# mratsim/constantine

Hardware: NVIDIA H100
Metric: bls12_381_g1_msm_throughput (higher is better)
Workload: dtype u32

## Files before the change

constantine_b200/csrc/msm_affine.cuh:

```cuda
#pragma once
#include "ec.cuh"
#include "field_inv.cuh"

namespace b200 {

constexpr int AFF_MAX_LEVELS = 8;
constexpr uint32_t AFF_NONE = 0xFFFFFFFFu;

static __global__ void k_bucket_bounds(const uint32_t* __restrict__ keys, size_t n, uint32_t no_key, uint32_t* head, uint32_t* tail) {
  size_t q = (size_t)blockIdx.x * blockDim.x + threadIdx.x;
  if (q >= n) return;
  const uint32_t key = keys[q];
  if (key >= no_key) return;
  if (q == 0 || keys[q - 1] != key) head[key] = (uint32_t)q;
  if (q + 1 == n || keys[q + 1] != key) tail[key] = (uint32_t)(q + 1);
}

constexpr int SCAN_THREADS = 256, SCAN_PER_THREAD = 4, SCAN_ITEMS = SCAN_THREADS * SCAN_PER_THREAD;

B200_DEV uint32_t block_exclusive_scan(uint32_t v, uint32_t& total, uint32_t* smem ) {
  const unsigned lane = threadIdx.x & 31u, warp = threadIdx.x >> 5;
  uint32_t inc = v;
#pragma unroll
  for (int d = 1; d < 32; d <<= 1) {
// ... 254 lines not shown
  else load_words_rw(x, src + (size_t)ref * (2 * T::WORDS));
  return x;
}
template <class T, bool FIRST>
B200_DEV T load_y(const uint32_t* src, uint32_t ref, bool& is_inf_if_x_zero) {
  T y;
  if constexpr (FIRST) {
    load_words(y, src + (size_t)(ref & 0x7FFFFFFFu) * (2 * T::WORDS) + T::WORDS);
    is_inf_if_x_zero = y.is_zero();
    y.cneg((ref >> 31) != 0);
  } else {
    load_words_rw(y, src + (size_t)ref * (2 * T::WORDS) + T::WORDS);
    is_inf_if_x_zero = y.is_zero();
  }
  return y;
}

template <class T>
B200_DEV int classify_pair(bool single, const T& x1, const T& y1, bool inf1, const T& x2, const T& y2, bool inf2, T& den) {
  if (single) return PAIR_COPY1;
  if (inf1) return PAIR_COPY2;
  if (inf2) return PAIR_COPY1;
  den = x2 - x1;
  if (!den.is_zero()) return PAIR_ADD;
  if (!(y1 == y2) || y1.is_zero()) return PAIR_INF;
  den = y1.dbl();
  return PAIR_DBL;
}

#ifndef B200_AFF_THREADS
#define B200_AFF_THREADS 128
#endif
#ifndef B200_AFF_MIN_BLOCKS
#define B200_AFF_MIN_BLOCKS 4
#endif

B200_DEV void prefetch_l2(const void* p) { asm volatile("prefetch.global.L2 [%0];" ::"l"(p)); }
B200_DEV void prefetch_span(const void* p, int bytes) {
  prefetch_l2(p);
  prefetch_l2((const char*)p + bytes - 1);
}
template <class T, bool FIRST>
B200_DEV void prefetch_point(const uint32_t* src, uint32_t ref) {
  const uint32_t idx = FIRST ? (ref & 0x7FFFFFFFu) : ref;
  prefetch_span(src + (size_t)idx * (2 * T::WORDS), 2 * T::WORDS * 4);
}

template <class T, bool FIRST>
__global__ void __launch_bounds__(B200_AFF_THREADS, (T::WORDS <= 12) ? B200_AFF_MIN_BLOCKS : 1)
k_affine_pairs(const void* __restrict__ plan, const uint32_t* __restrict__ total_ptr, const uint32_t* src, uint32_t* dst, uint4* scratch,
               const uint32_t* __restrict__ perm = nullptr, const uint32_t* __restrict__ range = nullptr) {
  const size_t threads = (size_t)gridDim.x * blockDim.x;
  const size_t tid = (size_t)blockIdx.x * blockDim.x + threadIdx.x;
  const uint32_t range_begin = range ? range[0] : 0u;
  const uint32_t total = range ? range[1] - range[0] : *total_ptr;
  if (perm) perm += range_begin;
  const uint32_t M = (uint32_t)(((size_t)total + threads - 1) / threads);
  const unsigned lane = threadIdx.x & 31u;
  const size_t warp_base = (tid - lane) * (size_t)M;
  if (warp_base >= total) return;
  uint32_t cnt = 0;
  {
    const size_t first = warp_base + lane;
    if (first < total) {
      const size_t left = (size_t)total - first;
      cnt = (uint32_t)((left + 31) / 32);
      if (cnt > M) cnt = M;
    }
  }
  T run = T::one();
  {
    auto slot_of = [&](size_t t) -> size_t { return perm ? (size_t)perm[t] : t; };
    PairTask t_next = cnt ? load_task<FIRST>(plan, slot_of(warp_base + lane)) : PairTask{0u, AFF_NONE};
    T x1n = T::zero(), x2n = T::zero();
    if (cnt) {
      x1n = load_x<T, FIRST>(src, t_next.a);
      if (t_next.b != AFF_NONE) x2n = load_x<T, FIRST>(src, t_next.b);
    }
#pragma unroll 1
    for (uint32_t j = 0; j < cnt; j++) {
      const PairTask t = t_next;
      const T x1 = x1n, x2 = x2n;
      if (j + 1 < cnt) {
        t_next = load_task<FIRST>(plan, slot_of(warp_base + lane + 32u * (size_t)(j + 1)));
        x1n = load_x<T, FIRST>(src, t_next.a);
        if (t_next.b != AFF_NONE) x2n = load_x<T, FIRST>(src, t_next.b);
      }
      const bool single = t.b == AFF_NONE;
      T den = x2 - x1;
      bool contributes = !single;
      if (!single && (den.is_zero() || x1.is_zero() || x2.is_zero())) {
        bool z1, z2;
        const T y1 = load_y<T, FIRST>(src, t.a, z1), y2 = load_y<T, FIRST>(src, t.b, z2);
        const int kind = classify_pair(false, x1, y1, z1 && x1.is_zero(), x2, y2, z2 && x2.is_zero(), den);
        contributes = kind >= PAIR_ADD;
      }
      if (contributes) run = run.mul_u(den);
      scratch_store(scratch, threads, tid, j, run);
    }
  }
  T inv = fe_inverse(run);
  auto slot_of2 = [&](size_t t) -> size_t { return perm ? (size_t)perm[t] : t; };
  size_t p_prev = cnt ? slot_of2(warp_base + lane + 32u * (size_t)(cnt - 1)) : 0;
  PairTask t_prev = cnt ? load_task<FIRST>(plan, p_prev) : PairTask{0u, AFF_NONE};
#pragma unroll 1
  for (uint32_t jj = cnt; jj > 0; jj--) {
    const uint32_t j = jj - 1;
    const size_t p = p_prev;
    const PairTask t = t_prev;
    if (j > 0) {
      p_prev = slot_of2(warp_base + lane + 32u * (size_t)(j - 1));
      t_prev = load_task<FIRST>(plan, p_prev);
      prefetch_point<T, FIRST>(src, t_prev.a);
      if (t_prev.b != AFF_NONE) prefetch_point<T, FIRST>(src, t_prev.b);
      if (j > 1) {
        constexpr int V = T::WORDS / 4;
#pragma unroll
        for (int k = 0; k < V; k++) prefetch_l2(scratch + ((size_t)(j - 2) * V + k) * threads + tid);
      }
    }
    const bool single = t.b == AFF_NONE;
    Aff<T> P1, P2;
    bool z1 = false, z2 = false;
    P1.x = load_x<T, FIRST>(src, t.a);
    P1.y = load_y<T, FIRST>(src, t.a, z1);
    if (!single) {
      P2.x = load_x<T, FIRST>(src, t.b);
      P2.y = load_y<T, FIRST>(src, t.b, z2);
    } else {
      P2.x = T::zero(); P2.y = T::zero();
    }
    T den;
    const int kind = classify_pair(single, P1.x, P1.y, z1 && P1.x.is_zero(), P2.x, P2.y, z2 && P2.x.is_zero(), den);
    Aff<T> R;
    if (kind < PAIR_ADD) {
      if (kind == PAIR_COPY1) R = P1;
      else if (kind == PAIR_COPY2) R = P2;
      else { R.x = T::zero(); R.y = T::zero(); }
    } else {
      T inv_den = inv;
      if (j > 0) inv_den = inv.mul_u(scratch_load<T>(scratch, threads, tid, j - 1));
      inv = inv.mul_u(den);
      T num;
      if (kind == PAIR_ADD) num = P2.y - P1.y;
      else { const T xx = P1.x.sqr(); num = xx.dbl() + xx; }
      const T lam = num.mul_u(inv_den);
      R.x = lam.sqr_u() - P1.x - P2.x;
      R.y = lam.mul_u(P1.x - R.x) - P1.y;
    }
    store_affine(dst, p, R);
  }
}

}
```

constantine_b200/csrc/msm_engine.cuh:

```cuda
#pragma once
#include <cstdio>
#include <cstdlib>
#include <cstring>
#include <atomic>
#include <condition_variable>
#include <functional>
#include <memory>
#include <mutex>
#include <thread>
#include <vector>
#include <cuda_runtime.h>
#include <cub/device/device_radix_sort.cuh>
#include <cub/device/device_scan.cuh>
#include "msm_kernels.cuh"
#include "msm_affine.cuh"
#include "host_field.hpp"

namespace b200 {

#define B200_CUDA_CHECK(expr)                                                                              \
  do {                                                                                                     \
    cudaError_t e__ = (expr);                                                                              \
    if (e__ != cudaSuccess) {                                                                              \
      fprintf(stderr, "[ctt_b200_msm] FATAL CUDA error %s (%s) at %s:%d -- no CPU fallback exists\n",      \
// ... 347 lines not shown
                                      const PointChunks* point_chunks = nullptr, bool batch_out_device = false) {
  using T = typename C::T;
  using H = typename C::H;
  using HP = host::HXyzz<H>;
  constexpr int KFIX = 32;
  Stats& st = E.stats;
  int launches = 0;
  if (batch == 0) return HP::inf();
  if (n == 0) {
    if (batch_out) for (size_t m = 0; m < batch; m++) batch_out[m] = HP::inf();
    return HP::inf();
  }
  if (batch * n >= (1ull << 31)) { fprintf(stderr, "[ctt_b200_msm] FATAL: len >= 2^31 unsupported\n"); abort(); }
  if (batch > 1 && (batch_out == nullptr || win_begin != 0 || win_end >= 0 || point_sets < 1 || point_sets > batch)) {
    fprintf(stderr, "[ctt_b200_msm] FATAL: a batch takes all windows and needs an output array\n"); abort();
  }
  const bool table_mode = table_stride > 0;
  if (input_chunks && (batch > 1 || table_mode || input_chunks->empty())) input_chunks = nullptr;

  int c = force_c > 0 ? force_c : (E.tuning.force_c > 0 ? E.tuning.force_c : choose_window(n, C::SCALAR_BITS, T::WORDS));
  if (c < 2) c = 2;
  if (c > 20) c = 20;
  DigitPlan plan = make_plan(C::SCALAR_BITS, c, win_begin, win_end);
  const int nwd = plan.win_end - plan.win_begin;
  if (nwd <= 0) return HP::inf();
  const int nws = table_mode ? 1 : nwd;
  const size_t nw_total = batch * (size_t)nws;
  if (table_mode && (size_t)nwd * table_stride >= (1ull << 31)) { fprintf(stderr, "[ctt_b200_msm] FATAL: table too large\n"); abort(); }
  const uint32_t B = plan.buckets_per_window;
  const size_t nbuckets = nw_total * B;
  if (nbuckets >= 0xFFFFFFF0ull || nw_total >= (1ull << 30) || (size_t)nwd * batch * n >= (1ull << 32)) {
    fprintf(stderr, "[ctt_b200_msm] FATAL: batch too large for 32-bit bucket keys\n"); abort();
  }
  const int nw = (int)nw_total;
  const uint32_t no_key = (uint32_t)nbuckets;
  constexpr size_t XYZZ_BYTES = 4 * T::WORDS * 4;
  constexpr size_t XW = 4 * T::WORDS;
  constexpr size_t AFF_BYTES = 2 * T::WORDS * 4;
  st.c = c; st.num_windows = nwd; st.total_buckets = nbuckets; st.ms_affine = 0; st.entries = 0; st.groups = 1;
#ifndef B200_INLINE_MAX_WORDS
#define B200_INLINE_MAX_WORDS 12
#endif
  constexpr bool INL = (T::WORDS <= B200_INLINE_MAX_WORDS);
  cudaStream_t s = E.compute();
  E.buckets.ensure(nbuckets * XYZZ_BYTES);
  if (E.collect_timing) B200_CUDA_CHECK(cudaEventRecord(E.ev[0], s));
  B200_CUDA_CHECK(cudaMemsetAsync(E.buckets.ptr, 0, nbuckets * XYZZ_BYTES, s));

  const std::vector<InputChunk> whole = {InputChunk{0, n, wait_points}};
  const std::vector<InputChunk>& chunks_in = input_chunks ? *input_chunks : whole;
  for (size_t ck = 0; ck < chunks_in.size(); ck++) {
    const InputChunk& ch = chunks_in[ck];
    if (ch.count == 0) continue;
    const bool into = ck > 0;
    const bool last_chunk = ck + 1 == chunks_in.size();
    const bool timed = E.collect_timing && last_chunk;
    const size_t nper = ch.count;
    const size_t ntot = batch * nper;
    const size_t entries = (size_t)nwd * ntot;
    const void* sc = (const char*)d_scalars + ch.begin * 32;
    const void* pts = table_mode ? d_points : (const void*)((const char*)d_points + ch.begin * AFF_BYTES);
    st.entries += entries;

    int AL = E.tuning.affine_levels;
    if (AL < 0) AL = auto_affine_levels(entries, nbuckets, batch, T::WORDS);
    if (entries >= (1ull << 31) || nbuckets >= (1ull << 30)) AL = 0;
    if (AL > AFF_MAX_LEVELS) AL = AFF_MAX_LEVELS;
    auto level_cap = [&](int r) { return (entries >> r) + nbuckets + 1; };
    const size_t acc_entries = AL ? level_cap(AL) : entries;
    int KACC = 64;
    uint32_t fit_threads;
    {
      static thread_local int acc_bps_cache[MAX_DEVICES] = {};
      int bps = acc_bps_cache[E.device];
      if (bps == 0) {
        B200_CUDA_CHECK(cudaOccupancyMaxActiveBlocksPerMultiprocessor(&bps, k_accumulate<T>, B200_ACC_THREADS, 0));
        if (bps < 1) bps = 1;
        acc_bps_cache[E.device] = bps;
      }
      fit_threads = (uint32_t)(E.sm_count * bps * B200_ACC_THREADS);
      if (E.tuning.slice_len > 0) { KACC = E.tuning.slice_len; fit_threads = 0; }
      else if (E.tuning.slice_len < 0) KACC = -E.tuning.slice_len;
    }
    st.slice_len = fit_threads ? accumulate_slice_len(acc_entries, fit_threads, KACC) : KACC;
    E.keys_a.ensure(entries * 4); E.keys_b.ensure(entries * 4);
    E.vals_a.ensure(entries * 4); E.vals_b.ensure(entries * 4);
    if (timed) B200_CUDA_CHECK(cudaEventRecord(E.ev[10], s));
    if (input_chunks && ch.ready) B200_CUDA_CHECK(cudaStreamWaitEvent(s, ch.ready, 0));
    {
      dim3 grid((unsigned)((ntot + 255) / 256)), block(256);
      const uint32_t msm_key_stride = (uint32_t)nws * B, psets = batch > 1 ? (uint32_t)point_sets : 1u;
      if (fr_mont)
        k_digits<typename C::FrParams, true><<<grid, block, 0, s>>>((const uint32_t*)sc, (uint32_t)ntot, plan, (uint32_t*)E.keys_a.ptr, (uint32_t*)E.vals_a.ptr,
                                                                     table_mode ? 0u : B, no_key, (uint32_t)table_stride, (uint32_t)nper, msm_key_stride, psets);
      else
        k_digits<typename C::FrParams, false><<<grid, block, 0, s>>>((const uint32_t*)sc, (uint32_t)ntot, plan, (uint32_t*)E.keys_a.ptr, (uint32_t*)E.vals_a.ptr,
                                                                      table_mode ? 0u : B, no_key, (uint32_t)table_stride, (uint32_t)nper, msm_key_stride, psets);
      launches++;
    }
    if (timed) B200_CUDA_CHECK(cudaEventRecord(E.ev[1], s));
    int end_bit = 1;
    while ((1ull << end_bit) <= (unsigned long long)no_key) end_bit++;
    cub::DoubleBuffer<uint32_t> dk((uint32_t*)E.keys_a.ptr, (uint32_t*)E.keys_b.ptr);
    cub::DoubleBuffer<uint32_t> dv((uint32_t*)E.vals_a.ptr, (uint32_t*)E.vals_b.ptr);
    {
      size_t tmp_bytes = 0;
      B200_CUDA_CHECK(cub::DeviceRadixSort::SortPairs(nullptr, tmp_bytes, dk, dv, (int64_t)entries, 0, end_bit, s));
      E.cub_tmp.ensure(tmp_bytes);
      B200_CUDA_CHECK(cub::DeviceRadixSort::SortPairs(E.cub_tmp.ptr, tmp_bytes, dk, dv, (int64_t)entries, 0, end_bit, s));
      launches += 2 + (end_bit + 7) / 8;
    }
    const uint32_t* keys = dk.Current();
    const uint32_t* vals = dv.Current();
    if (timed) B200_CUDA_CHECK(cudaEventRecord(E.ev[2], s));
    E.bounds.ensure((size_t)(nw + 1) * 8);
    k_window_bounds<<<(unsigned)((nw + 1 + 63) / 64), 64, 0, s>>>(keys, entries, B, nw, (unsigned long long*)E.bounds.ptr);
    launches++;
    size_t max_slices;
    {
      size_t set_cap = table_mode ? (size_t)nwd * nper : nper;
      if (AL) set_cap = (set_cap >> AL) + B + 1;
      const size_t list_cap = (size_t)nw * set_cap;
      max_slices = fit_threads ? accumulate_waves(list_cap, fit_threads, KACC) * fit_threads : (list_cap + KACC - 1) / KACC;
    }
    const size_t max_fix = (max_slices + KFIX - 1) / KFIX;
    E.part_pts[0].ensure(max_slices * XYZZ_BYTES); E.part_keys[0].ensure(max_slices * 4);
    E.part_pts[1].ensure(max_fix * XYZZ_BYTES); E.part_keys[1].ensure(max_fix * 4);
    const int PC = (point_chunks && !input_chunks) ? point_chunks->P : 0;
    auto piece_ready = [&](int q) {
      if (point_chunks->stage && *point_chunks->stage) (*point_chunks->stage)(q);
      B200_CUDA_CHECK(cudaStreamWaitEvent(s, point_chunks->ready[q], 0));
    };
    auto wait_for_points = [&]() {
      if (PC) { for (int q = 0; q < PC; q++) piece_ready(q); }
      else if (!input_chunks && ch.ready) B200_CUDA_CHECK(cudaStreamWaitEvent(s, ch.ready, 0));
    };
    const void* acc_points = pts;
    if (AL) {
      const uint32_t nb = (uint32_t)nbuckets;
      const uint32_t nblk = (nb + SCAN_ITEMS - 1) / SCAN_ITEMS;
      const size_t off_stride = (size_t)nb + 1;
      E.aff_head.ensure((size_t)nb * 4); E.aff_tail.ensure((size_t)nb * 4);
      E.aff_off.ensure((size_t)(AL + 1) * off_stride * 4);
      E.aff_blocksum.ensure((size_t)(AL + 1) * nblk * 4);
      E.aff_plan[0].ensure(level_cap(1) * 8);
      for (int r = 1; r < AL; r++) E.aff_plan[r].ensure(level_cap(r + 1) * 4);
      E.aff_work[1].ensure(level_cap(1) * AFF_BYTES);
      if (AL >= 2) E.aff_work[0].ensure(level_cap(2) * AFF_BYTES);
      E.keys_s.ensure(acc_entries * 4);
      E.vals_s.ensure(acc_entries * 4);
      static thread_local int bps_cache[MAX_DEVICES] = {};
      int bps = bps_cache[E.device];
      if (bps == 0) {
        B200_CUDA_CHECK(cudaOccupancyMaxActiveBlocksPerMultiprocessor(&bps, k_affine_pairs<T, true>, B200_AFF_THREADS, 0));
        int bps2 = 0;
        B200_CUDA_CHECK(cudaOccupancyMaxActiveBlocksPerMultiprocessor(&bps2, k_affine_pairs<T, false>, B200_AFF_THREADS, 0));
        if (bps2 < bps) bps = bps2;
        if (bps < 1) bps = 1;
        bps_cache[E.device] = bps;
      }
      const unsigned aff_grid = (unsigned)(E.sm_count * bps);
      const size_t aff_threads = (size_t)aff_grid * B200_AFF_THREADS;
      const size_t per_thread = (level_cap(1) + aff_threads - 1) / aff_threads;
      E.aff_scratch.ensure(per_thread * aff_threads * (size_t)T::WORDS * 4);
      uint32_t* head = (uint32_t*)E.aff_head.ptr;
      uint32_t* tail = (uint32_t*)E.aff_tail.ptr;
      uint32_t* off = (uint32_t*)E.aff_off.ptr;
      B200_CUDA_CHECK(cudaMemsetAsync(head, 0, (size_t)nb * 4, s));
      B200_CUDA_CHECK(cudaMemsetAsync(tail, 0, (size_t)nb * 4, s));
      B200_CUDA_CHECK(cudaMemsetAsync(E.keys_s.ptr, 0xFF, acc_entries * 4, s));
      const unsigned eb = (unsigned)((entries + 255) / 256);
      k_bucket_bounds<<<eb, 256, 0, s>>>(keys, entries, no_key, head, tail);
      k_level_blocksums<<<nblk, SCAN_THREADS, 0, s>>>(head, tail, nb, AL, nblk, (uint32_t*)E.aff_blocksum.ptr);
      k_level_scan<<<1, SCAN_THREADS, 0, s>>>((uint32_t*)E.aff_blocksum.ptr, nblk, AL, nb, off);
      k_level_offsets<<<nblk, SCAN_THREADS, 0, s>>>(head, tail, nb, AL, nblk, (const uint32_t*)E.aff_blocksum.ptr, off);
      AffinePlan aplan;
      aplan.plan0 = (uint2*)E.aff_plan[0].ptr;
      for (int r = 0; r < AFF_MAX_LEVELS; r++) aplan.plan[r] = (r >= 1 && r < AL) ? (uint32_t*)E.aff_plan[r].ptr : nullptr;
      aplan.surv_keys = (uint32_t*)E.keys_s.ptr;
      aplan.surv_vals = (uint32_t*)E.vals_s.ptr;
      k_affine_plan<<<eb, 256, 0, s>>>(keys, vals, entries, no_key, head, tail, off, nb, AL, aplan);
      const bool split0 = PC > 1;
      if (!split0) wait_for_points();
      for (int r = 0; r < AL; r++) {
        const uint32_t* total_ptr = off + (size_t)(r + 1) * off_stride + nb;
        uint32_t* dst = (uint32_t*)E.aff_work[(r + 1) & 1].ptr;
        if (r == 0 && split0) {
          const uint32_t Pq = (uint32_t)PC;
          const uint32_t nblk_p = (uint32_t)((level_cap(1) + PART_TILE - 1) / PART_TILE);
          E.part_counts.ensure((size_t)Pq * nblk_p * 4);
          E.part_starts.ensure((size_t)(Pq + 1) * 4);
          E.part_perm.ensure(level_cap(1) * 4);
          k_part_count<<<nblk_p, PART_THREADS, 0, s>>>((const uint2*)E.aff_plan[0].ptr, total_ptr, (uint32_t)nper, Pq, nblk_p, (uint32_t*)E.part_counts.ptr);
          k_part_scan<<<1, SCAN_THREADS, 0, s>>>((uint32_t*)E.part_counts.ptr, Pq, nblk_p, (uint32_t*)E.part_starts.ptr);
          k_part_scatter<<<nblk_p, PART_THREADS, 0, s>>>((const uint2*)E.aff_plan[0].ptr, total_ptr, (uint32_t)nper, Pq, nblk_p,
                                                          (const uint32_t*)E.part_counts.ptr, (uint32_t*)E.part_perm.ptr);
          for (int q = 0; q < PC; q++) {
            piece_ready(q);
            k_affine_pairs<T, true><<<aff_grid, B200_AFF_THREADS, 0, s>>>(E.aff_plan[0].ptr, total_ptr, (const uint32_t*)pts, dst, (uint4*)E.aff_scratch.ptr,
                                                                          (const uint32_t*)E.part_perm.ptr, (const uint32_t*)E.part_starts.ptr + q);
          }
          launches += 3 + PC - 1;
        } else if (r == 0)
          k_affine_pairs<T, true><<<aff_grid, B200_AFF_THREADS, 0, s>>>(E.aff_plan[0].ptr, total_ptr, (const uint32_t*)pts, dst, (uint4*)E.aff_scratch.ptr);
        else
          k_affine_pairs<T, false><<<aff_grid, B200_AFF_THREADS, 0, s>>>(E.aff_plan[r].ptr, total_ptr, (const uint32_t*)E.aff_work[r & 1].ptr, dst, (uint4*)E.aff_scratch.ptr);
      }
      keys = (const uint32_t*)E.keys_s.ptr;
      vals = (const uint32_t*)E.vals_s.ptr;
      acc_points = E.aff_work[AL & 1].ptr;
      k_window_bounds<<<(unsigned)((nw + 1 + 63) / 64), 64, 0, s>>>(keys, acc_entries, B, nw, (unsigned long long*)E.bounds.ptr);
      launches += 6 + AL;
      B200_CUDA_CHECK(cudaGetLastError());
      if (timed) B200_CUDA_CHECK(cudaEventRecord(E.ev[9], s));
    }
    st.affine_levels = AL;
    if (!AL) wait_for_points();
    {
      dim3 block(B200_ACC_THREADS), grid((unsigned)((max_slices + B200_ACC_THREADS - 1) / B200_ACC_THREADS));
      k_accumulate<T><<<grid, block, 0, s>>>(keys, vals, (const unsigned long long*)E.bounds.ptr, 0, nw, no_key, (const uint32_t*)acc_points,
                                             (uint32_t*)E.buckets.ptr, (uint32_t*)E.part_pts[0].ptr, (uint32_t*)E.part_keys[0].ptr, max_slices, KACC,
                                             into ? 1 : 0, fit_threads);
      launches++;
    }
    if (timed) B200_CUDA_CHECK(cudaEventRecord(E.ev[3], s));
    {
      size_t count = max_slices;
      int cur = 0;
      while (count > 1) {
        size_t ns = (count + KFIX - 1) / KFIX;
        dim3 block(128), grid((unsigned)((count + 127) / 128));
        k_fixup<T><<<grid, block, 0, s>>>((const uint32_t*)E.part_keys[cur].ptr, (const uint32_t*)E.part_pts[cur].ptr, count,
                                          (uint32_t*)E.buckets.ptr, (uint32_t*)E.part_pts[cur ^ 1].ptr, (uint32_t*)E.part_keys[cur ^ 1].ptr);
        launches++;
        count = ns;
        cur ^= 1;
      }
    }
    if (timed) B200_CUDA_CHECK(cudaEventRecord(E.ev[4], s));
  }

  const bool plane_reduce = (batch == 1 && E.tuning.reduce_mode == 0);
  const int pr_a = (c - 1) / 2, pr_rbits = (c - 1) - pr_a;
  const uint32_t pr_planes = (uint32_t)(c - 1);
  const uint32_t pr_groups = (pr_planes + 3) / 4;
  uint32_t row = 0;
  DeviceBuffer* src = &E.red_a;
  if (plane_reduce) {
    const uint32_t Cn = 1u << pr_a, Rn = 1u << pr_rbits;
#ifndef B200_REDUCE_THREADS_PER_SM
#define B200_REDUCE_THREADS_PER_SM 256
#endif
    const size_t want_threads = (size_t)E.sm_count * B200_REDUCE_THREADS_PER_SM;
    uint32_t serial = 2;
    while (serial < 64 && nbuckets / (size_t)serial >= want_threads) serial *= 2;
    constexpr uint32_t MAX_LANES = T::WORDS >= 12 ? 128u : 32u;
    auto lanes_for = [&](uint32_t len) { uint32_t l = len / serial; if (l < 1) l = 1; if (l > MAX_LANES) l = MAX_LANES; return (int)l; };
    const int lanes_r = lanes_for(Cn), lanes_c = lanes_for(Rn);
    E.red_a.ensure((size_t)nw * Rn * XYZZ_BYTES);
    E.red_b.ensure((size_t)nw * Cn * XYZZ_BYTES);
    E.red_planes.ensure((size_t)nw * (pr_planes + pr_groups) * XYZZ_BYTES);
    const size_t tr = (size_t)nw * Rn * lanes_r, tc = (size_t)nw * Cn * lanes_c;
    const unsigned row_blocks = (unsigned)((tr + 127) / 128), col_blocks = (unsigned)((tc + 127) / 128);
    k_rowcol_sums<T, INL><<<row_blocks + col_blocks, 128, 0, s>>>((const uint32_t*)E.buckets.ptr, B, pr_a, (uint32_t)nw, lanes_r, lanes_c, row_blocks,
                                                                  (uint32_t*)E.red_a.ptr, (uint32_t*)E.red_b.ptr);
    const int lanes_p = (MAX_LANES > 32 && (Rn >= 128 || Cn >= 128)) ? 128 : 32;
    const size_t tp = (size_t)nw * pr_planes * lanes_p;
    uint32_t* planes_ptr = (uint32_t*)E.red_planes.ptr;
    uint32_t* digits_ptr = planes_ptr + (size_t)nw * pr_planes * XW;
    k_plane_sums<T, INL><<<(unsigned)((tp + 127) / 128), 128, 0, s>>>((const uint32_t*)E.red_a.ptr, (const uint32_t*)E.red_b.ptr, pr_a, pr_rbits,
                                                                      (uint32_t)nw, lanes_p, planes_ptr);
    k_plane_combine<T, INL><<<(unsigned)(((size_t)nw * pr_groups * 4 + 63) / 64), 64, 0, s>>>(planes_ptr, pr_planes, pr_groups, (uint32_t)nw, digits_ptr);
    launches += 3;
  } else {
    uint32_t L = (uint32_t)E.tuning.reduce_chunk;
    if (L < 1) L = 1;
    uint32_t chunks = (B + L - 1) / L;
    const size_t want_threads = (size_t)E.sm_count * 64;
    while (L > 1 && (size_t)chunks * nw < want_threads && chunks < B) { L = (L + 1) / 2; chunks = (B + L - 1) / L; }
    int nbits = 0;
    while (nbits < 32 && ((uint64_t)(chunks - 1) * L >> nbits) != 0) nbits++;
    E.red_a.ensure((size_t)chunks * nw * XYZZ_BYTES);
    E.red_b.ensure((size_t)chunks * nw * XYZZ_BYTES);
    size_t threads = (size_t)chunks * nw;
    dim3 block(64), grid((unsigned)((threads + 63) / 64));
    k_bucket_reduce<T, INL><<<grid, block, 0, s>>>((const uint32_t*)E.buckets.ptr, B, L, chunks, (uint32_t)nw, (uint32_t*)E.red_a.ptr, (uint32_t*)E.red_b.ptr);
    k_chunk_offset<T, INL><<<grid, block, 0, s>>>((uint32_t*)E.red_a.ptr, (const uint32_t*)E.red_b.ptr, L, chunks, (uint32_t)nw, nbits);
    launches += 2;
    row = chunks;
    bool in_a = true;
    const uint32_t row_stop = batch > 1 ? 1u : 4u;
    while (row > row_stop) {
      uint32_t out_row = (row + 31) / 32;
      size_t warps = (size_t)out_row * nw;
      dim3 blk(128), grd((unsigned)((warps * 32 + 127) / 128));
      k_row_sum_warp<T, INL><<<grd, blk, 0, s>>>((const uint32_t*)(in_a ? E.red_a.ptr : E.red_b.ptr), row, out_row, (uint32_t)nw,
                                                 (uint32_t*)(in_a ? E.red_b.ptr : E.red_a.ptr));
      launches++;
      row = out_row;
      in_a = !in_a;
    }
    src = in_a ? &E.red_a : &E.red_b;
  }
  if (E.collect_timing) B200_CUDA_CHECK(cudaEventRecord(E.ev[5], s));
  static_assert(sizeof(HP) == XYZZ_BYTES, "host/device XYZZ layout");
  if (d_digits_out) {
    if (!plane_reduce) { fprintf(stderr, "[ctt_b200_msm] FATAL: device digits need the bit-plane reduction (single MSM, reduce mode 0)\n"); abort(); }
    B200_CUDA_CHECK(cudaMemcpyAsync(d_digits_out, (const uint32_t*)E.red_planes.ptr + (size_t)nw * pr_planes * XW, (size_t)nw * pr_groups * XYZZ_BYTES,
                                    cudaMemcpyDeviceToDevice, s));
    st.kernel_launches = launches;
    st.ms_total = 0;
    return HP::inf();
  }
  auto read_times = [&]() {
    if (!E.collect_timing) return;
    B200_CUDA_CHECK(cudaEventRecord(E.ev[6], s));
    B200_CUDA_CHECK(cudaEventSynchronize(E.ev[6]));
    collect_msm_times(E);
  };
  if (batch > 1 && batch_out_device) {
    k_batch_tail<T><<<(unsigned)((batch + 63) / 64), 64, 0, s>>>((const uint32_t*)src->ptr, row, nws, c, (uint32_t)batch, (uint32_t*)batch_out);
    launches++;
    if (E.collect_timing) B200_CUDA_CHECK(cudaEventRecord(E.ev[6], s));
    st.kernel_launches = launches;
    return HP::inf();
  }
  if (batch > 1) {
    DeviceBuffer* dst = (src == &E.red_a) ? &E.red_b : &E.red_a;
    k_batch_tail<T><<<(unsigned)((batch + 63) / 64), 64, 0, s>>>((const uint32_t*)src->ptr, row, nws, c, (uint32_t)batch, (uint32_t*)dst->ptr);
    launches++;
    E.ensure_host(batch * XYZZ_BYTES);
    B200_CUDA_CHECK(cudaMemcpyAsync(E.h_result, dst->ptr, batch * XYZZ_BYTES, cudaMemcpyDeviceToHost, s));
    B200_CUDA_CHECK(cudaStreamSynchronize(s));
    memcpy((void*)batch_out, E.h_result, batch * XYZZ_BYTES);
    read_times();
    st.kernel_launches = launches;
    return HP::inf();
  }
  HP r = HP::inf();
  if (plane_reduce) {
    const size_t out_bytes = (size_t)nw * pr_groups * XYZZ_BYTES;
    E.ensure_host(out_bytes);
    B200_CUDA_CHECK(cudaMemcpyAsync(E.h_result, (const uint32_t*)E.red_planes.ptr + (size_t)nw * pr_planes * XW, out_bytes, cudaMemcpyDeviceToHost, s));
    B200_CUDA_CHECK(cudaStreamSynchronize(s));
    r = horner_window_digits<H>(reinterpret_cast<const HP*>(E.h_result), nw, (int)pr_groups, c, table_mode ? 0 : plan.win_begin);
  } else {
    const size_t out_bytes = (size_t)nw * row * XYZZ_BYTES;
    E.ensure_host(out_bytes);
    B200_CUDA_CHECK(cudaMemcpyAsync(E.h_result, src->ptr, out_bytes, cudaMemcpyDeviceToHost, s));
    B200_CUDA_CHECK(cudaStreamSynchronize(s));
    const HP* parts = reinterpret_cast<const HP*>(E.h_result);
    auto window_sum = [&](int w) {
      HP a = parts[(size_t)w * row];
      for (uint32_t i = 1; i < row; i++) a = host::xyzz_add(a, parts[(size_t)w * row + i]);
      return a;
    };
    r = window_sum(nw - 1);
    for (int w = nw - 2; w >= 0; w--) {
      for (int i = 0; i < c; i++) r = host::xyzz_dbl(r);
// ... 446 lines not shown
```

Before: 101.5.

## Add warp-specialized producer/consumer affine pair kernel with cp.async ring buffers

```diff
diff --git a/constantine_b200/csrc/msm_affine.cuh b/constantine_b200/csrc/msm_affine.cuh
--- a/constantine_b200/csrc/msm_affine.cuh
+++ b/constantine_b200/csrc/msm_affine.cuh
@@ -430,4 +430,272 @@
   }
 }
 
-}
+#ifndef B200_AFF_WS_CONSUMERS
+#define B200_AFF_WS_CONSUMERS 8
+#endif
+#ifndef B200_AFF_WS_STAGES
+#define B200_AFF_WS_STAGES 2
+#endif
+constexpr int AFF_WS_CONSUMERS = B200_AFF_WS_CONSUMERS;
+constexpr int AFF_WS_THREADS = 32 * (AFF_WS_CONSUMERS + 1);
+
+template <class T>
+struct AffRing {
+  static constexpr bool USED = T::WORDS <= 12;
+  static constexpr int V = T::WORDS / 4;
+  static constexpr int S2 = B200_AFF_WS_STAGES;
+  static constexpr int ROWS = S2 * 5 * V;
+  static constexpr int S1 = ROWS / (2 * V);
+  static constexpr size_t BYTES = (size_t)AFF_WS_CONSUMERS * ROWS * 32 * 16;
+};
+
+B200_DEV uint32_t smem_addr(const void* p) { return (uint32_t)__cvta_generic_to_shared(p); }
+B200_DEV void mbar_init(uint64_t* b, uint32_t count) { asm volatile("mbarrier.init.shared::cta.b64 [%0], %1;" ::"r"(smem_addr(b)), "r"(count) : "memory"); }
+B200_DEV void mbar_arrive(uint64_t* b) { asm volatile("mbarrier.arrive.shared::cta.b64 _, [%0];" ::"r"(smem_addr(b)) : "memory"); }
+B200_DEV void mbar_wait(uint64_t* b, uint32_t parity) {
+  asm volatile(
+      "{\n\t.reg .pred P1;\n"
+      "WAIT:\n\t"
+      "mbarrier.try_wait.parity.shared::cta.b64 P1, [%0], %1;\n\t"
+      "@!P1 bra WAIT;\n\t}" ::"r"(smem_addr(b)),
+      "r"(parity)
+      : "memory");
+}
+B200_DEV void cp_async_arrive(uint64_t* b) { asm volatile("cp.async.mbarrier.arrive.noinc.shared::cta.b64 [%0];" ::"r"(smem_addr(b)) : "memory"); }
+B200_DEV void cp_async16(void* s, const void* g) { asm volatile("cp.async.cg.shared.global [%0], [%1], 16;" ::"r"(smem_addr(s)), "l"(g) : "memory"); }
+
+template <class T>
+B200_DEV void ring_fetch(uint4* ring, int row, unsigned lane, const uint32_t* g) {
+#pragma unroll
+  for (int k = 0; k < T::WORDS / 4; k++) cp_async16(ring + (row + k) * 32 + lane, g + 4 * k);
+}
+template <class T>
+B200_DEV T ring_load(const uint4* ring, int row, unsigned lane) {
+  T v;
+#pragma unroll
+  for (int k = 0; k < T::WORDS / 4; k++) {
+    const uint4 w = ring[(row + k) * 32 + lane];
+    v.set_word(4 * k + 0, w.x); v.set_word(4 * k + 1, w.y); v.set_word(4 * k + 2, w.z); v.set_word(4 * k + 3, w.w);
+  }
+  return v;
+}
+
+template <class T, bool FIRST>
+__global__ void __launch_bounds__(AFF_WS_THREADS, 1)
+k_affine_pairs_ws(const void* __restrict__ plan, const uint32_t* __restrict__ total_ptr, const uint32_t* src, uint32_t* dst, uint4* scratch,
+                  const uint32_t* __restrict__ perm = nullptr, const uint32_t* __restrict__ range = nullptr) {
+  using RG = AffRing<T>;
+  constexpr int V = RG::V, NC = AFF_WS_CONSUMERS, S1 = RG::S1, S2 = RG::S2;
+  extern __shared__ __align__(16) unsigned char aff_ring_raw[];
+  __shared__ uint64_t full1[NC][S1], empty1[NC][S1], full2[NC][S2], empty2[NC][S2], drained[NC];
+  __shared__ uint32_t s_task[NC][S1][3][32];
+  const unsigned lane = threadIdx.x & 31u, warp = threadIdx.x >> 5;
+  if (threadIdx.x == 0) {
+    for (int w = 0; w < NC; w++) {
+      for (int s = 0; s < S1; s++) { mbar_init(&full1[w][s], 64); mbar_init(&empty1[w][s], 32); }
+      for (int s = 0; s < S2; s++) { mbar_init(&full2[w][s], 64); mbar_init(&empty2[w][s], 32); }
+      mbar_init(&drained[w], 32);
+    }
+  }
+  __syncthreads();
+  const size_t threads = (size_t)gridDim.x * NC * 32;
+  const uint32_t range_begin = range ? range[0] : 0u;
+  const uint32_t total = range ? range[1] - range[0] : *total_ptr;
+  if (perm) perm += range_begin;
+  const uint32_t M = (uint32_t)(((size_t)total + threads - 1) / threads);
+  auto count_of = [&](size_t tid) -> uint32_t {
+    const size_t first = (tid & ~(size_t)31) * M + (tid & 31u);
+    if (first >= total) return 0u;
+    const uint32_t c = (uint32_t)(((size_t)total - first + 31) / 32);
+    return c < M ? c : M;
+  };
+  auto slot_at = [&](size_t tid, uint32_t j) -> size_t {
+    const size_t t = (tid & ~(size_t)31) * M + (tid & 31u) + 32u * (size_t)j;
+    return perm ? (size_t)perm[t] : t;
+  };
+  uint4* const ring_base = reinterpret_cast<uint4*>(aff_ring_raw);
+
+  if (warp == NC) {
+    uint32_t n[NC], cnt[NC];
+#pragma unroll
+    for (int w = 0; w < NC; w++) {
+      const size_t tid = ((size_t)blockIdx.x * NC + w) * 32 + lane;
+      n[w] = count_of(tid - lane);
+      cnt[w] = count_of(tid);
+    }
+    auto tid_of = [&](int w) { return ((size_t)blockIdx.x * NC + w) * 32 + lane; };
+    auto src_of = [&](uint32_t ref) { return src + (size_t)(FIRST ? (ref & 0x7FFFFFFFu) : ref) * (2 * T::WORDS); };
+    uint32_t ta[NC], tb[NC], tp[NC];
+    auto fetch_task = [&](int w, uint32_t j) {
+      const size_t p = slot_at(tid_of(w), j);
+      const PairTask t = load_task<FIRST>(plan, p);
+      ta[w] = t.a; tb[w] = t.b; tp[w] = (uint32_t)p;
+    };
+#pragma unroll
+    for (int w = 0; w < NC; w++) if (cnt[w]) fetch_task(w, 0);
+#pragma unroll 1
+    for (uint32_t j = 0; j < n[0]; j++) {
+      uint32_t ca[NC], cb[NC];
+#pragma unroll
+      for (int w = 0; w < NC; w++) { ca[w] = ta[w]; cb[w] = tb[w]; }
+#pragma unroll
+      for (int w = 0; w < NC; w++) if (j + 1 < cnt[w]) fetch_task(w, j + 1);
+#pragma unroll
+      for (int w = 0; w < NC; w++) {
+        if (j >= n[w]) continue;
+        const int s = (int)(j % S1);
+        mbar_wait(&empty1[w][s], ((j / S1) & 1u) ^ 1u);
+        uint4* ring = ring_base + (size_t)w * RG::ROWS * 32;
+        if (j < cnt[w]) {
+          s_task[w][s][0][lane] = ca[w];
+          s_task[w][s][1][lane] = cb[w];
+          ring_fetch<T>(ring, s * 2 * V, lane, src_of(ca[w]));
+          if (cb[w] != AFF_NONE) ring_fetch<T>(ring, s * 2 * V + V, lane, src_of(cb[w]));
+        }
+        cp_async_arrive(&full1[w][s]);
+        mbar_arrive(&full1[w][s]);
+      }
+    }
+#pragma unroll
+    for (int w = 0; w < NC; w++) if (n[w] && n[w] - 1 < cnt[w]) fetch_task(w, n[w] - 1);
+#pragma unroll 1
+    for (uint32_t jj = 0; jj < n[0]; jj++) {
+      uint32_t ca[NC], cb[NC], cp[NC];
+#pragma unroll
+      for (int w = 0; w < NC; w++) { ca[w] = ta[w]; cb[w] = tb[w]; cp[w] = tp[w]; }
+#pragma unroll
+      for (int w = 0; w < NC; w++) if (jj + 1 < n[w] && n[w] - 2 - jj < cnt[w]) fetch_task(w, n[w] - 2 - jj);
+#pragma unroll
+      for (int w = 0; w < NC; w++) {
+        if (jj >= n[w]) continue;
+        if (jj == 0) mbar_wait(&drained[w], 0);
+        const uint32_t j = n[w] - 1 - jj;
+        const int s = (int)(jj % S2);
+        mbar_wait(&empty2[w][s], ((jj / S2) & 1u) ^ 1u);
+        uint4* ring = ring_base + (size_t)w * RG::ROWS * 32;
+        if (j < cnt[w]) {
+          s_task[w][s][0][lane] = ca[w];
+          s_task[w][s][1][lane] = cb[w];
+          s_task[w][s][2][lane] = cp[w];
+          const int row = s * 5 * V;
+          ring_fetch<T>(ring, row, lane, src_of(ca[w]));
+          ring_fetch<T>(ring, row + V, lane, src_of(ca[w]) + T::WORDS);
+          if (cb[w] != AFF_NONE) {
+            ring_fetch<T>(ring, row + 2 * V, lane, src_of(cb[w]));
+            ring_fetch<T>(ring, row + 3 * V, lane, src_of(cb[w]) + T::WORDS);
+          }
+          if (j > 0) {
+#pragma unroll
+            for (int k = 0; k < V; k++)
+              cp_async16(ring + (row + 4 * V + k) * 32 + lane, scratch + ((size_t)(j - 1) * V + k) * threads + tid_of(w));
+          }
+        }
+        cp_async_arrive(&full2[w][s]);
+        mbar_arrive(&full2[w][s]);
+      }
+    }
+    asm volatile("cp.async.wait_all;" ::: "memory");
+    return;
+  }
+
+  const size_t tid = ((size_t)blockIdx.x * NC + warp) * 32 + lane;
+  const uint32_t n = count_of(tid - lane), cnt = count_of(tid);
+  if (n == 0) return;
+  const uint4* ring = ring_base + (size_t)warp * RG::ROWS * 32;
+  T run = T::one();
+#pragma unroll 1
+  for (uint32_t j = 0; j < n; j++) {
+    const int s = (int)(j % S1);
+    mbar_wait(&full1[warp][s], (j / S1) & 1u);
+    const uint32_t a = s_task[warp][s][0][lane], b = s_task[warp][s][1][lane];
+    const T x1 = ring_load<T>(ring, s * 2 * V, lane), x2 = ring_load<T>(ring, s * 2 * V + V, lane);
+    mbar_arrive(&empty1[warp][s]);
+    if (j >= cnt) continue;
+    const bool single = b == AFF_NONE;
+    T den = x2 - x1;
+    bool contributes = !single;
+    if (!single && (den.is_zero() || x1.is_zero() || x2.is_zero())) {
+      bool z1, z2;
+      const T y1 = load_y<T, FIRST>(src, a, z1), y2 = load_y<T, FIRST>(src, b, z2);
+      const int kind = classify_pair(false, x1, y1, z1 && x1.is_zero(), x2, y2, z2 && x2.is_zero(), den);
+      contributes = kind >= PAIR_ADD;
+    }
+    if (contributes) run = run.mul_u(den);
+    scratch_store(scratch, threads, tid, j, run);
+  }
+  mbar_arrive(&drained[warp]);
+  T inv = fe_inverse(run);
+#pragma unroll 1
+  for (uint32_t jj = 0; jj < n; jj++) {
+    const uint32_t j = n - 1 - jj;
+    const int s = (int)(jj % S2);
+    mbar_wait(&full2[warp][s], (jj / S2) & 1u);
+    const int row = s * 5 * V;
+    const uint32_t a = s_task[warp][s][0][lane], b = s_task[warp][s][1][lane], p = s_task[warp][s][2][lane];
+    const bool single = b == AFF_NONE;
+    Aff<T> P1, P2;
+    P1.x = ring_load<T>(ring, row, lane);
+    P1.y = ring_load<T>(ring, row + V, lane);
+    P2.x = single ? T::zero() : ring_load<T>(ring, row + 2 * V, lane);
+    P2.y = single ? T::zero() : ring_load<T>(ring, row + 3 * V, lane);
+    const T pre = ring_load<T>(ring, row + 4 * V, lane);
+    mbar_arrive(&empty2[warp][s]);
+    if (j >= cnt) continue;
+    const bool z1 = P1.y.is_zero(), z2 = P2.y.is_zero();
+    if constexpr (FIRST) {
+      P1.y.cneg((a >> 31) != 0);
+      if (!single) P2.y.cneg((b >> 31) != 0);
+    }
+    T den;
+    const int kind = classify_pair(single, P1.x, P1.y, z1 && P1.x.is_zero(), P2.x, P2.y, z2 && P2.x.is_zero(), den);
+    Aff<T> R;
+    if (kind < PAIR_ADD) {
+      if (kind == PAIR_COPY1) R = P1;
+      else if (kind == PAIR_COPY2) R = P2;
+      else { R.x = T::zero(); R.y = T::zero(); }
+    } else {
+      T inv_den = inv;
+      if (j > 0) inv_den = inv.mul_u(pre);
+      inv = inv.mul_u(den);
+      T num;
+      if (kind == PAIR_ADD) num = P2.y - P1.y;
+      else { const T xx = P1.x.sqr(); num = xx.dbl() + xx; }
+      const T lam = num.mul_u(inv_den);
+      R.x = lam.sqr_u() - P1.x - P2.x;
+      R.y = lam.mul_u(P1.x - R.x) - P1.y;
+    }
+    store_affine(dst, p, R);
+  }
+}
+
+template <class T>
+constexpr int affine_pairs_slot_threads() { return AffRing<T>::USED ? 32 * AFF_WS_CONSUMERS : B200_AFF_THREADS; }
+
+template <class T>
+cudaError_t affine_pairs_blocks_per_sm(int* bps) {
+  int b1 = 0, b2 = 0;
+  cudaError_t e;
+  if constexpr (AffRing<T>::USED) {
+    constexpr int bytes = (int)AffRing<T>::BYTES;
+    if ((e = cudaFuncSetAttribute(k_affine_pairs_ws<T, true>, cudaFuncAttributeMaxDynamicSharedMemorySize, bytes)) != cudaSuccess) return e;
+    if ((e = cudaFuncSetAttribute(k_affine_pairs_ws<T, false>, cudaFuncAttributeMaxDynamicSharedMemorySize, bytes)) != cudaSuccess) return e;
+    if ((e = cudaOccupancyMaxActiveBlocksPerMultiprocessor(&b1, k_affine_pairs_ws<T, true>, AFF_WS_THREADS, bytes)) != cudaSuccess) return e;
+    if ((e = cudaOccupancyMaxActiveBlocksPerMultiprocessor(&b2, k_affine_pairs_ws<T, false>, AFF_WS_THREADS, bytes)) != cudaSuccess) return e;
+  } else {
+    if ((e = cudaOccupancyMaxActiveBlocksPerMultiprocessor(&b1, k_affine_pairs<T, true>, B200_AFF_THREADS, 0)) != cudaSuccess) return e;
+    if ((e = cudaOccupancyMaxActiveBlocksPerMultiprocessor(&b2, k_affine_pairs<T, false>, B200_AFF_THREADS, 0)) != cudaSuccess) return e;
+  }
+  *bps = b2 < b1 ? b2 : b1;
+  return cudaSuccess;
+}
+
+template <class T, bool FIRST>
+void launch_affine_pairs(unsigned grid, cudaStream_t s, const void* plan, const uint32_t* total_ptr, const uint32_t* src, uint32_t* dst, uint4* scratch,
+                         const uint32_t* perm = nullptr, const uint32_t* range = nullptr) {
+  if constexpr (AffRing<T>::USED)
+    k_affine_pairs_ws<T, FIRST><<<grid, AFF_WS_THREADS, AffRing<T>::BYTES, s>>>(plan, total_ptr, src, dst, scratch, perm, range);
+  else
+    k_affine_pairs<T, FIRST><<<grid, B200_AFF_THREADS, 0, s>>>(plan, total_ptr, src, dst, scratch, perm, range);
+}
+
+}
diff --git a/constantine_b200/csrc/msm_engine.cuh b/constantine_b200/csrc/msm_engine.cuh
--- a/constantine_b200/csrc/msm_engine.cuh
+++ b/constantine_b200/csrc/msm_engine.cuh
@@ -523,15 +523,12 @@
       static thread_local int bps_cache[MAX_DEVICES] = {};
       int bps = bps_cache[E.device];
       if (bps == 0) {
-        B200_CUDA_CHECK(cudaOccupancyMaxActiveBlocksPerMultiprocessor(&bps, k_affine_pairs<T, true>, B200_AFF_THREADS, 0));
-        int bps2 = 0;
-        B200_CUDA_CHECK(cudaOccupancyMaxActiveBlocksPerMultiprocessor(&bps2, k_affine_pairs<T, false>, B200_AFF_THREADS, 0));
-        if (bps2 < bps) bps = bps2;
+        B200_CUDA_CHECK(affine_pairs_blocks_per_sm<T>(&bps));
         if (bps < 1) bps = 1;
         bps_cache[E.device] = bps;
       }
       const unsigned aff_grid = (unsigned)(E.sm_count * bps);
-      const size_t aff_threads = (size_t)aff_grid * B200_AFF_THREADS;
+      const size_t aff_threads = (size_t)aff_grid * affine_pairs_slot_threads<T>();
       const size_t per_thread = (level_cap(1) + aff_threads - 1) / aff_threads;
       E.aff_scratch.ensure(per_thread * aff_threads * (size_t)T::WORDS * 4);
       uint32_t* head = (uint32_t*)E.aff_head.ptr;
@@ -568,14 +565,14 @@
                                                           (const uint32_t*)E.part_counts.ptr, (uint32_t*)E.part_perm.ptr);
           for (int q = 0; q < PC; q++) {
             piece_ready(q);
-            k_affine_pairs<T, true><<<aff_grid, B200_AFF_THREADS, 0, s>>>(E.aff_plan[0].ptr, total_ptr, (const uint32_t*)pts, dst, (uint4*)E.aff_scratch.ptr,
-                                                                          (const uint32_t*)E.part_perm.ptr, (const uint32_t*)E.part_starts.ptr + q);
+            launch_affine_pairs<T, true>(aff_grid, s, E.aff_plan[0].ptr, total_ptr, (const uint32_t*)pts, dst, (uint4*)E.aff_scratch.ptr,
+                                         (const uint32_t*)E.part_perm.ptr, (const uint32_t*)E.part_starts.ptr + q);
           }
           launches += 3 + PC - 1;
         } else if (r == 0)
-          k_affine_pairs<T, true><<<aff_grid, B200_AFF_THREADS, 0, s>>>(E.aff_plan[0].ptr, total_ptr, (const uint32_t*)pts, dst, (uint4*)E.aff_scratch.ptr);
+          launch_affine_pairs<T, true>(aff_grid, s, E.aff_plan[0].ptr, total_ptr, (const uint32_t*)pts, dst, (uint4*)E.aff_scratch.ptr);
         else
-          k_affine_pairs<T, false><<<aff_grid, B200_AFF_THREADS, 0, s>>>(E.aff_plan[r].ptr, total_ptr, (const uint32_t*)E.aff_work[r & 1].ptr, dst, (uint4*)E.aff_scratch.ptr);
+          launch_affine_pairs<T, false>(aff_grid, s, E.aff_plan[r].ptr, total_ptr, (const uint32_t*)E.aff_work[r & 1].ptr, dst, (uint4*)E.aff_scratch.ptr);
       }
       keys = (const uint32_t*)E.keys_s.ptr;
       vals = (const uint32_t*)E.vals_s.ptr;
```

New measurement: 105.3 (median of 6 runs). 1.04x the previous value.
